# bkomuves/plonky2-verifier

Hardware: AMD Instinct MI355X
Metric: Plonky2 proofs verified/sec (std config, 28 FRI queries) at 1/2/4/8 MI355X (higher is better)
Workload: dtype u64 (Goldilocks mod-p integer)

## Files before the change

plonky2-verifier_amd/csrc/api_internal.hpp:

```cpp
#pragma once
#include <hip/hip_runtime.h>
#include <atomic>
#include <memory>
#include <mutex>
#include <string>
#include <utility>
#include <vector>
#include "../../include/p2v.h"
#include "circuit.hpp"
#include "dev.h"

using namespace p2v;

#pragma GCC visibility push(hidden)
extern thread_local std::string g_err;
inline int fail(int code, const std::string& msg) { g_err = msg; return code; }

template <class F>
int guarded(int other, F fn) {
  try { fn(); return P2V_OK; }
  catch (const ShapeError& e) { return fail(P2V_E_SHAPE, e.what()); }
  catch (const ParseError& e) { return fail(P2V_E_PARSE, e.what()); }
  catch (const CircuitError& e) { return fail(P2V_E_CIRCUIT, e.what()); }
  catch (const std::exception& e) { return fail(other, e.what()); }
// ... 65 lines not shown
  mutable std::vector<HostPipe*> pool;
  mutable std::mutex known_mu;
  mutable std::vector<std::unique_ptr<KnownTable>> known;
  ~p2v_circuit();
};

struct p2v_verifier {
  const p2v_circuit* circ = nullptr;
  int device = 0;
  size_t max_batch = 0, Bmax = 0;
  DevCircuit dc{};
  size_t in_bytes = 0;
  std::atomic<bool> p1_recorded{false};
  p2v_verifier* chain_prev = nullptr;
  std::vector<p2v_verifier*> chain_next;
  unsigned la_seq = 0;
  float last_ms[kNumKernels] = {0};
  bool timed = false;
  int transcript_mode = 0;
  int quad_min_batch = 4096;
  int lane_min_batch = 16384;
  bool merkle_cse = true;
  bool cse_dirty = false;
  int known_mode = 1;
  const KnownTable* known = nullptr;
  bool known_dirty = false;
  int lat_max_batch = 64;
  bool single_stream = false;
  bool debug_sync = false;
  ProofTemplate tmpl;
  bool have_tmpl = false;
  int64_t skel_len = 0, ntok = 0;
  bool have_bmap = false;
  int nruns = 0, nchk = 0;
  int64_t bfixed = 0;

  PinnedBuf h_res;
  Event ev[2 * kNumKernels];
  Event dep_p1, dep_side, dep_fri, dep_v3;
  Event p1_done;
  Event tr_done[2], chal_free[2];
  Stream side;
  Stream side2;
  Stream ts;
  Stream side3;
  DevBuf kid;
// ... 44 lines not shown
```

plonky2-verifier_amd/csrc/api_run.cpp:

```cpp
#include <algorithm>
#include <cstdio>
#include <cstring>
#include "api_internal.hpp"
#include "kernels.h"

extern "C" {

size_t p2v_tiled_words(size_t n, size_t proof_words) { return (n + 63) / 64 * 64 * proof_words; }

void p2v_tile_proofs(const uint64_t* pm, size_t n, size_t W, uint64_t* tiled) {
  if (!pm || !tiled) return;
  const size_t tiles = (n + 63) / 64;
  for (size_t t = 0; t < tiles; t++) {
    uint64_t* dst = tiled + t * W * 64;
    for (size_t w = 0; w < W; w++)
      for (size_t l = 0; l < 64; l++) {
        const size_t i = t * 64 + l;
        dst[w * 64 + l] = i < n ? pm[i * W + w] : 0;
      }
  }
}

static void launch_phase1(const DevCircuit& d, int tl, int nt_blocks, int leaf_blocks, hipStream_t s) {
  auto* k = d.key_id ? (tl == 1 ? k_phase1_lane_keyed : k_phase1_keyed) : (tl == 1 ? k_phase1_lane : k_phase1);
  k<<<nt_blocks + leaf_blocks, 256, 0, s>>>(d, nt_blocks, tl);
}
static void launch_transcript(const DevCircuit& d, int tl, int nt_blocks, hipStream_t s) {
  auto* k = d.key_id ? (tl == 1 ? k_transcript_lane_keyed : k_transcript_keyed) : (tl == 1 ? k_transcript_lane : k_transcript);
  k<<<nt_blocks, 256, 0, s>>>(d, tl);
}
static void launch_vanish(void (*k)(DevCircuit), int first, int last, int NPB, hipStream_t s, const DevCircuit& d) {
  k<<<(last - first) * NPB, 64, 0, s>>>(d);
}

int p2v_verifier_run(p2v_verifier* v, const uint64_t* proofs, size_t n, int8_t* results, uint64_t* trace, void* stream_, uint32_t flags) {
  return p2v_verifier_run_keyed(v, proofs, nullptr, n, results, trace, stream_, flags);
}

int p2v_verifier_run_keyed(p2v_verifier* v, const uint64_t* proofs, const uint32_t* key_ids, size_t n, int8_t* results,
                           uint64_t* trace, void* stream_, uint32_t flags) {
  if (!v || (!proofs && n) || !results) return fail(P2V_E_ARG, "null argument");
  if (n > v->max_batch) return fail(P2V_E_ARG, "batch larger than max_batch");
  if (n == 0) return P2V_OK;
  HCK(hipSetDevice(v->device));
  hipStream_t st = (hipStream_t)stream_;
  const Circuit& C = v->circ->c;
  DevCircuit d = v->dc;
  d.n = (int)n;
// ... 28 lines not shown
  d.soa = src;
  int tl = d.B >= v->lane_min_batch ? 1 : d.B >= v->quad_min_batch ? 4 : 16;
  if (v->transcript_mode == 1) tl = 16;
  else if (v->transcript_mode == 2) tl = 4;
  else if (v->transcript_mode == 3) tl = 1;
  const int nt_blocks = (tl * d.B + 255) / 256;
  const bool lat = d.n <= v->lat_max_batch;
  const bool key_rows = !key_ids || (d.nkeys > 1 && v->known && v->known->kkeys == d.nkeys);
  if (v->known && key_rows && !lat && d.mcse) {
    d.kmode = v->known_mode; d.kskip = 1;
    int k = 0;
    for (int j = 0; j < d.T; j++) if (v->dc.leaf_order[j] != 0) d.leaf_order[k++] = v->dc.leaf_order[j];
    d.nleaf = k;
  }
  const int leaf_units = d.Q * d.nleaf * NPB;
  bool chained = false;
  {
    std::lock_guard<std::mutex> lk(g_chain_mu);
    chained = v->chain_prev != nullptr;
    if (v->chain_prev && v->chain_prev->p1_recorded.load(std::memory_order_acquire))
      HCK(hipStreamWaitEvent(st, v->chain_prev->p1_done, 0));
  }
  const bool la = (flags & P2V_FLAG_LOOKAHEAD) && (flags & P2V_FLAG_INPUT_DEVICE) && sd != st && !chained;
  int la_slot = 0;
  if (la) {
    if (!v->ts) HCK(v->ts.create());
    la_slot = (int)(v->la_seq++ & 1u);
    d.chal = (uint64_t*)(la_slot ? v->chal2.p : v->chal.p);
    HCK(hipStreamWaitEvent(v->ts, v->chal_free[la_slot], 0));
    T0(SLOT_TRANSCRIPT, v->ts);
    launch_transcript(d, tl, nt_blocks, v->ts);
    DBG("k_transcript", v->ts);
    T1(SLOT_TRANSCRIPT, v->ts);
    HCK(hipEventRecord(v->tr_done[la_slot], v->ts));
    T0(SLOT_LEAF, st);
    k_leaf<<<(leaf_units + 3) / 4, 256, 0, st>>>(d);
    DBG("k_leaf", st);
    T1(SLOT_LEAF, st);
    HCK(hipStreamWaitEvent(st, v->tr_done[la_slot], 0));
    HCK(hipEventRecord(v->dep_p1, st));
    HCK(hipStreamWaitEvent(sd, v->dep_p1, 0));
  } else {
    T0(SLOT_PHASE1, st);
    launch_phase1(d, tl, nt_blocks, (leaf_units + 3) / 4, st);
    DBG("k_phase1", st);
    T1(SLOT_PHASE1, st);
    if (sd != st) {
      HCK(hipEventRecord(v->dep_p1, st));
      HCK(hipStreamWaitEvent(sd, v->dep_p1, 0));
    }
  }
  HCK(hipEventRecord(v->p1_done, st));
  v->p1_recorded.store(true, std::memory_order_release);
  const int mk_wg = lat ? 64 : 256;
  const bool fri2 = lat && sd != st;
  if (fri2 && !v->side2) HCK(v->side2.create());
  if (fri2) {
    HCK(hipStreamWaitEvent(v->side2, v->p1_done, 0));
    T0(SLOT_FRI, v->side2);
    k_fri<<<(d.Q * NPB * 64 + mk_wg - 1) / mk_wg, mk_wg, 0, v->side2>>>(d);
    DBG("k_fri", v->side2);
    T1(SLOT_FRI, v->side2);
    HCK(hipEventRecord(v->dep_fri, v->side2));
  }
  if (d.kmode) {
    if (v->known_dirty) HCK(hipMemsetAsync(v->k_missn.p, 0, 64, sd));
    v->known_dirty = true;
// ... 27 lines not shown
    HCK(hipEventRecord(v->dep_v3, sv));
    HCK(hipStreamWaitEvent(sd, v->dep_v3, 0));
  }
  if (d.vcls[4] > d.vcls[3]) launch_vanish(r2 ? k_vanish_lookup_r2 : k_vanish_lookup_rn, d.vcls[3], d.vcls[4], NPB, sd, d);
  DBG("k_vanish_lookup", sd);
  if (d.vcls[5] > d.vcls[4]) launch_vanish(r2 ? k_vanish_prog_r2 : k_vanish_prog_rn, d.vcls[4], d.vcls[5], NPB, sd, d);
  DBG("k_vanish_prog", sd);
  T1(SLOT_VANISH, sd);
  T0(SLOT_VANISH_FINAL, sd);
  k_vanish_final<<<(d.B + 255) / 256, 256, 0, sd>>>(d);
  DBG("k_vanish_final", sd);
  T1(SLOT_VANISH_FINAL, sd);
  if (!fri2) {
    T0(SLOT_FRI, sd);
    k_fri<<<(d.Q * NPB * 64 + 255) / 256, 256, 0, sd>>>(d);
    DBG("k_fri", sd);
    T1(SLOT_FRI, sd);
  }
  if (sd != st) HCK(hipEventRecord(v->dep_side, sd));
  T0(SLOT_MERKLE, st);
  const int merkle_units = d.Q * d.T * NPB;
  if (lat) k_merkle_row<<<(unsigned)(((int64_t)d.Q * d.T * d.n * 16 + 255) / 256), 256, 0, st>>>(d);
  else if (d.mcse) {
    const int ncls = 1 + d.S;
    if (v->cse_dirty) HCK(hipMemsetAsync(v->m_count.p, 0, (size_t)(d.depth0 + 2) * 64, st));
    v->cse_dirty = true;
    k_merkle_plan<<<(ncls * d.Q * NPB + P2V_PLAN_WAVES - 1) / P2V_PLAN_WAVES, 64 * P2V_PLAN_WAVES, 0, st>>>(d);
    DBG("k_merkle_plan", st);
    const int64_t cse_waves = ((int64_t)(d.T - d.kskip) * d.Q * d.n + 63) / 64 + d.depth0 + 1;
    k_merkle_cse<<<(unsigned)((cse_waves + 31) / 32 * 8), 256, 0, st>>>(d);
    DBG("k_merkle_cse", st);
    k_merkle_fix<<<P2V_FIX_BLOCKS, 256, 0, st>>>(d);
    DBG("k_merkle_fix", st);
    k_merkle_resolve<<<(d.Q * (d.T - d.kskip) * NPB + 3) / 4, 256, 0, st>>>(d);
    DBG("k_merkle_resolve", st);
    v->cse_dirty = false;
  } else k_merkle<<<(merkle_units + 3) / 4, 256, 0, st>>>(d);
  DBG("k_merkle", st);
  T1(SLOT_MERKLE, st);
  if (sd != st) HCK(hipStreamWaitEvent(st, v->dep_side, 0));
  if (fri2) HCK(hipStreamWaitEvent(st, v->dep_fri, 0));
  T0(SLOT_STATUS, st);
  k_status<<<(unsigned)((n + 255) / 256), 256, 0, st>>>(d, dres, dtrace, C.trace_words);
  DBG("k_status", st);
  T1(SLOT_STATUS, st);
  v->known_dirty = false;
  if (la) HCK(hipEventRecord(v->chal_free[la_slot], st));
  else if (sd != st) HCK(hipEventRecord(v->chal_free[0], st));
#undef T0
#undef T1
#undef DBG
// ... 29 lines not shown
```

plonky2-verifier_amd/csrc/api_workspace.cpp:

```cpp
#include <algorithm>
#include <cstdlib>
#include <cstring>
#include "api_internal.hpp"
#include "gl.h"
#include "poseidon_constants.h"

std::mutex g_chain_mu;


void fill_scalars(const Circuit& C, DevCircuit& d) {
  d.r = C.r; d.Q = C.num_queries; d.S = (int)C.arities.size(); d.T = 4 + d.S;
  d.num_pis = C.num_pis; d.cap_len = C.cap_len; d.degree_bits = C.degree_bits; d.lde_bits = C.lde_bits; d.pow_bits = C.pow_bits;
  d.num_wires = C.num_wires; d.num_routed = C.num_routed; d.num_constants = C.num_constants; d.ngc = C.num_gate_consts;
  d.ngroups = (int)C.grp_start.size(); d.nls = C.nls; d.nlp = C.nlp; d.npp = C.npp; d.qdf = C.qdf; d.nluts = (int)C.lut_in.size();
  d.depth0 = C.depth0; d.final_len = C.final_len;
  for (int t = 0; t < 4; t++) { d.width[t] = C.oracle_width[t]; d.lwidth[t] = C.leaf_width[t]; }
  d.noop_leaves = C.noop_leaves ? 1 : 0;
  d.n_gates = C.n_gate_eval; d.n_pp_terms = (int)C.n_pp_terms_per_round; d.n_lookup_terms = (int)C.n_lookup_terms_per_round;
  d.alpha_base_gates = C.alpha_base_gates;
  d.prog_pih = -1;
  const Layout& L = C.L;
  d.pis = L.pis; d.wcap = L.wcap; d.zcap = L.zcap; d.qcap = L.qcap; d.o_const = L.o_const; d.o_sig = L.o_sig; d.o_wires = L.o_wires;
  d.o_zs = L.o_zs; d.o_pp = L.o_pp; d.o_quot = L.o_quot; d.o_lzs = L.o_lzs; d.o_zs_next = L.o_zs_next; d.o_lzs_next = L.o_lzs_next;
  d.n_this = L.n_this; d.n_next = L.n_next; d.ccaps = L.ccaps; d.final_poly = L.final_poly; d.pow = L.pow; d.q0 = L.q0; d.qstride = L.qstride;
// ... 192 lines not shown
  }
  v->chain_prev = prev;
  if (prev) prev->chain_next.push_back(v);
  return P2V_OK;
}

int p2v_verifier_create(const p2v_circuit* pc, int device, size_t max_batch, p2v_verifier** out) {
  if (!pc || !out || max_batch == 0) return fail(P2V_E_ARG, "null argument / zero batch");
  if (const char* tm = getenv("P2V_TRANSCRIPT"); tm && !strcmp(tm, "pair"))
    return fail(P2V_E_ARG, "P2V_TRANSCRIPT=pair: the pair transcript form was retired (DESIGN.md §5.7)");
  int ndev = 0;
  if (hipGetDeviceCount(&ndev) != hipSuccess || ndev == 0) return fail(P2V_E_NODEVICE, "no HIP device available: libp2v verifies on MI355X only (no CPU fallback)");
  if (device < 0 || device >= ndev) return fail(P2V_E_ARG, "bad device index");
  HCK(hipSetDevice(device));
  const Circuit& C = pc->c;
  VerifierPtr v(new p2v_verifier());
  v->circ = pc; v->device = device; v->max_batch = max_batch;
  v->Bmax = (max_batch + 63) / 64 * 64;
  if (const char* ss = getenv("P2V_SINGLE_STREAM")) v->single_stream = ss[0] == '1';
  if (const char* ds = getenv("P2V_DEBUG_SYNC")) v->debug_sync = ds[0] == '1';
  if (const char* lm = getenv("P2V_LANE_MIN")) v->lane_min_batch = atoi(lm) > 0 ? atoi(lm) : v->lane_min_batch;
  if (const char* qm = getenv("P2V_QUAD_MIN")) v->quad_min_batch = atoi(qm) > 0 ? atoi(qm) : v->quad_min_batch;
  if (const char* mc = getenv("P2V_MERKLE_CSE")) v->merkle_cse = mc[0] != '0';
  if (const char* kl = getenv("P2V_KNOWN_LEAVES")) v->known_mode = kl[0] == '0' ? 0 : kl[0] == '2' ? 2 : 1;
  if (const char* lx = getenv("P2V_LAT_MAX")) v->lat_max_batch = atoi(lx) >= 0 ? atoi(lx) : v->lat_max_batch;
  if (const char* tm = getenv("P2V_TRANSCRIPT")) v->transcript_mode = !strcmp(tm, "row") ? 1 : !strcmp(tm, "quad") ? 2 : !strcmp(tm, "lane") ? 3 : 0;
  DevCircuit& d = v->dc;
  memset(&d, 0, sizeof d);
  fill_scalars(C, d);
  const CircuitTables t = circuit_tables(C);
  d.n_lut_pieces = t.pbase.back();
#define ACK(x) HCK_AS("device allocation", x)
  {
    std::vector<uint64_t> keys(C.cs_cap);
    keys.insert(keys.end(), C.digest, C.digest + 4);
    keys.insert(keys.end(), C.extra_keys.begin(), C.extra_keys.end());
    keys.insert(keys.end(), 8, 0);
    ACK(upload(v->t_cs, keys, d.keys));
    d.cs_cap = d.keys;
    d.nkeys = (int32_t)C.num_keys();
  }
  ACK(v->kid.alloc(v->Bmax * sizeof(uint32_t)));
  ACK(upload(v->t_kis, C.k_is, d.k_is));
  ACK(upload(v->t_gkind, t.gkind, d.gate_kind)); ACK(upload(v->t_gpar, t.gpar, d.gate_par)); ACK(upload(v->t_ggrp, t.ggrp, d.gate_grp));
  ACK(upload(v->t_gwoff, t.gwoff, d.gate_woff)); ACK(upload(v->t_w, t.wts, d.weights)); ACK(upload(v->t_gs, t.gs, d.grp_start)); ACK(upload(v->t_ge, t.ge, d.grp_end));
  ACK(upload(v->t_lin, t.lin, d.lut_in)); ACK(upload(v->t_lout, t.lout, d.lut_out)); ACK(upload(v->t_loff, t.loff, d.lut_off)); ACK(upload(v->t_llen, t.llen, d.lut_len));
// ... 85 lines not shown
```

plonky2-verifier_amd/csrc/dev.h:

```cpp
#pragma once
#include <stdint.h>

#define P2V_MAX_STEPS 8
#define P2V_MAX_R 4
#define P2V_LUT_CHUNK 16
#define P2V_LUT_PIECE 256
#define P2V_PLAN_WAVES 16
#define P2V_FIX_BLOCKS 256

struct DevCircuit {
  int32_t B;
  int32_t n;
  int32_t r, Q, S, T;
  int32_t num_pis, cap_len, degree_bits, lde_bits, pow_bits;
  int32_t num_wires, num_routed, num_constants, ngc, ngroups, nls, nlp, npp, qdf, nluts;
  int32_t depth0, final_len;
  int32_t arity[P2V_MAX_STEPS], step_depth[P2V_MAX_STEPS], step_logn[P2V_MAX_STEPS];
  int32_t width[4];
  int32_t lwidth[4];
  int32_t noop_leaves;
  int32_t tiled;
  int64_t wstride;
  int8_t leaf_order[4 + P2V_MAX_STEPS], merkle_order[4 + P2V_MAX_STEPS];
  int32_t n_gates;
  int32_t unit_filters;
  int32_t n_pp_terms, n_lookup_terms;
  int64_t alpha_base_gates;
  int64_t pis, wcap, zcap, qcap, o_const, o_sig, o_wires, o_zs, o_pp, o_quot, o_lzs, o_zs_next, o_lzs_next;
  int64_t n_this, n_next, ccaps, final_poly, pow, q0, qstride;
  int64_t leaf[4], path[4], step_evals[P2V_MAX_STEPS], step_path[P2V_MAX_STEPS];
// ... 123 lines not shown
```

plonky2-verifier_amd/csrc/kernels.h:

```cpp
#pragma once
#include <hip/hip_runtime.h>
#include <cstdint>
#include "dev.h"

extern "C" __global__ void k_phase1(DevCircuit, int, int);
extern "C" __global__ void k_phase1_lane(DevCircuit, int, int);
extern "C" __global__ void k_transcript(DevCircuit, int);
extern "C" __global__ void k_transcript_lane(DevCircuit, int);
extern "C" __global__ void k_phase1_keyed(DevCircuit, int, int);
extern "C" __global__ void k_phase1_lane_keyed(DevCircuit, int, int);
extern "C" __global__ void k_transcript_keyed(DevCircuit, int);
extern "C" __global__ void k_transcript_lane_keyed(DevCircuit, int);
extern "C" __global__ void k_leaf(DevCircuit);
extern "C" __global__ void k_fri(DevCircuit);
extern "C" __global__ void k_status(DevCircuit, int8_t*, uint64_t*, int64_t);
extern "C" __global__ void k_selftest(int, const uint64_t*, const uint64_t*, uint64_t*, int64_t);
extern "C" __global__ void k_selftest_forms(int, const uint64_t*, uint64_t*, int64_t);
extern "C" __global__ void k_selftest_field(int, DevCircuit, const uint64_t*, uint64_t*);
extern "C" __global__ void k_merkle(DevCircuit);
extern "C" __global__ void k_merkle_row(DevCircuit);
extern "C" __global__ void k_merkle_plan(DevCircuit);
extern "C" __global__ void k_merkle_cse(DevCircuit);
extern "C" __global__ void k_merkle_fix(DevCircuit);
extern "C" __global__ void k_merkle_resolve(DevCircuit);
extern "C" __global__ void k_merkle_known(DevCircuit);
extern "C" __global__ void k_merkle_known_miss(DevCircuit);
extern "C" __global__ void k_vanish_r2(DevCircuit);
extern "C" __global__ void k_vanish_rn(DevCircuit);
extern "C" __global__ void k_vanish_poseidon_r2(DevCircuit);
extern "C" __global__ void k_vanish_poseidon_rn(DevCircuit);
extern "C" __global__ void k_vanish_coset_r2(DevCircuit);
extern "C" __global__ void k_vanish_coset_rn(DevCircuit);
extern "C" __global__ void k_vanish_lookup_r2(DevCircuit);
// ... 12 lines not shown
```

plonky2-verifier_amd/csrc/kernels.hip:

```cpp
#include "leafhash.h"
#include "kernels.h"

using namespace p2d;
using gl::E;

__device__ __forceinline__ void leaf_hash_unit(const DevCircuit& c, int unit, int lane) {
  const int NPB = c.B >> 6;
  const int pb = unit % NPB, qt = unit / NPB;
  const int q = qt % c.Q, t = c.leaf_order[qt / c.Q];
  const int p = pb * 64 + lane;
  const int64_t base = c.q0 + (int64_t)q * c.qstride;
  int64_t off; int len;
  if (t < 4) { off = base + c.leaf[t]; len = c.lwidth[t]; }
  else { int s = t - 4; off = base + c.step_evals[s]; len = 2 << c.arity[s]; }
  uint64_t st[12];
  leaf_sponge(c, off, len, p, st);
  uint64_t* dst = c.leafdig + ((int64_t)(q * c.T + t) * 4) * c.B + p;
#pragma unroll
  for (int i = 0; i < 4; i++) dst[(int64_t)i * c.B] = st[i];
}

template <int D>
__device__ __forceinline__ uint64_t row_up(uint64_t v, bool plus) {
  const uint32_t lo = (uint32_t)v, hi = (uint32_t)(v >> 32);
// ... 166 lines not shown
      uint64_t w = f.get_word(x, outpos);
      outpos--;
      if (type == TOP_SQUEEZE_IDX) w &= qmask;
      if (a + k == CH_FRI_ALPHA(c)) fa0 = w;
      if (a + k == CH_FRI_ALPHA(c) + 1) fa1 = w;
      if (leader) chal(c, a + k, p) = w;
    }
  }
  E ap[F::LOG + 1] = {E{fa0, fa1}};
#pragma unroll
  for (int s = 1; s <= F::LOG; s++) ap[s] = gl::emul(ap[s - 1], ap[s - 1]);
  E H[2];
#pragma unroll
  for (int b = 0; b < 2 * F::SUMS_FIRST; b++) H[b] = horner_strided<1 << F::LOG>(c, b == 0 ? c.o_const : c.o_zs_next, b == 0 ? c.n_this : c.n_next, f.t, p, ap[F::LOG]);
#pragma unroll
  for (int b = 0; b < 2; b++) {
    if constexpr (!F::SUMS_FIRST) H[b] = horner_strided<1 << F::LOG>(c, b == 0 ? c.o_const : c.o_zs_next, b == 0 ? c.n_this : c.n_next, f.t, p, ap[F::LOG]);
    const E y = f.fold(H[b], ap);
    if (leader) { chal(c, (b == 0 ? CH_Y0(c) : CH_Y1(c)), p) = y.a; chal(c, (b == 0 ? CH_Y0(c) : CH_Y1(c)) + 1, p) = y.b; }
  }
}

template <int FORM = 0, bool KEYED = false>
__device__ __forceinline__ void transcript_block(const DevCircuit& c, int tl, TLdsAny& U) {
  const int g = blockIdx.x * 256 + threadIdx.x;
  if constexpr (FORM == 1) {
    if (g < c.B) transcript<KEYED>(c, g, LaneForm{});
  } else if (tl == 16) {
    lp::Row LR;
    lp::init(LR, U.l, threadIdx.x);
    if ((g >> 4) < c.B) transcript<KEYED>(c, g >> 4, RowForm(LR, U.l));
  } else {
    if ((g >> 2) < c.B) transcript<KEYED>(c, g >> 2, QuadForm{g & 3, U.q});
  }
}

template <int FORM, bool KEYED = false>
__device__ __forceinline__ void phase1_body(const DevCircuit& c, int nt_blocks, int tl) {
  const int lane = threadIdx.x & 63, wave = threadIdx.x >> 6;
  __shared__ TLdsAny T;
  if ((int)blockIdx.x < nt_blocks) {
    __builtin_amdgcn_s_setprio(3);
    if constexpr (FORM == 0) tlds_fill_form(T, tl);
    transcript_block<FORM, KEYED>(c, tl, T);
    return;
  }
  const int unit = ((int)blockIdx.x - nt_blocks) * 4 + wave;
  const int units = c.Q * c.nleaf * (c.B >> 6);
  if (unit < units) leaf_hash_unit(c, unit, lane);
}
extern "C" __global__ void __launch_bounds__(256) __attribute__((amdgpu_waves_per_eu(4))) k_phase1(DevCircuit c, int nt_blocks, int tl) {
  phase1_body<0>(c, nt_blocks, tl);
}
extern "C" __global__ void __launch_bounds__(256) __attribute__((amdgpu_waves_per_eu(4))) k_phase1_lane(DevCircuit c, int nt_blocks, int tl) {
  phase1_body<1>(c, nt_blocks, tl);
}
extern "C" __global__ void __launch_bounds__(256) __attribute__((amdgpu_waves_per_eu(4))) k_phase1_keyed(DevCircuit c, int nt_blocks, int tl) {
  phase1_body<0, true>(c, nt_blocks, tl);
}
extern "C" __global__ void __launch_bounds__(256) __attribute__((amdgpu_waves_per_eu(4))) k_phase1_lane_keyed(DevCircuit c, int nt_blocks, int tl) {
  phase1_body<1, true>(c, nt_blocks, tl);
}

extern "C" __global__ void __launch_bounds__(256) k_transcript(DevCircuit c, int tl) {
  __builtin_amdgcn_s_setprio(3);
  __shared__ TLdsAny T;
  tlds_fill_form(T, tl);
  transcript_block(c, tl, T);
}
extern "C" __global__ void __launch_bounds__(256) k_transcript_lane(DevCircuit c, int tl) {
  __builtin_amdgcn_s_setprio(3);
  __shared__ TLdsAny T;
  transcript_block<1>(c, tl, T);
}
extern "C" __global__ void __launch_bounds__(256) k_transcript_keyed(DevCircuit c, int tl) {
  __builtin_amdgcn_s_setprio(3);
  __shared__ TLdsAny T;
  tlds_fill_form(T, tl);
  transcript_block<0, true>(c, tl, T);
}
extern "C" __global__ void __launch_bounds__(256) k_transcript_lane_keyed(DevCircuit c, int tl) {
  __builtin_amdgcn_s_setprio(3);
  __shared__ TLdsAny T;
  transcript_block<1, true>(c, tl, T);
// ... 358 lines not shown
```

plonky2-verifier_amd/csrc/merkle.hip:

```cpp
#include "leafhash.h"
#include "kernels.h"

using namespace p2d;

__device__ __forceinline__ uint32_t entry_pack(int t, int q, int p) { return (uint32_t)t << 27 | (uint32_t)q << 22 | (uint32_t)p; }
__device__ __forceinline__ void entry_unpack(uint32_t id, int& t, int& q, int& p) {
  t = (int)(id >> 27); q = (int)((id >> 22) & 31); p = (int)(id & 0x3FFFFFu);
}
__device__ __forceinline__ uint32_t plan_pack(int e, int owner, bool same_leaf, int root) {
  return (uint32_t)e | (uint32_t)owner << 4 | (uint32_t)same_leaf << 9 | (uint32_t)root << 10;
}
__device__ __forceinline__ int plan_e(uint32_t pw) { return (int)(pw & 15); }
__device__ __forceinline__ int plan_owner(uint32_t pw) { return (int)((pw >> 4) & 31); }
__device__ __forceinline__ bool plan_same_leaf(uint32_t pw) { return (pw >> 9) & 1; }
__device__ __forceinline__ int plan_root(uint32_t pw) { return (int)((pw >> 10) & 31); }
__device__ __forceinline__ uint8_t& mk_at(const DevCircuit& c, int t, int q, int p) { return c.mk_ok[(int64_t)(q * c.T + t) * c.B + p]; }

#ifndef P2V_MERKLE_WAVES
#define P2V_MERKLE_WAVES 6
#endif
#if P2V_MERKLE_WAVES > 0
#define P2V_MERKLE_ATTR __attribute__((amdgpu_waves_per_eu(P2V_MERKLE_WAVES)))
#else
#define P2V_MERKLE_ATTR
#endif
__device__ __forceinline__ void tree_path(const DevCircuit& c, int t, int q, int p, int& depth, int64_t& poff, uint32_t& idx) {
  const int64_t base = c.q0 + (int64_t)q * c.qstride;
  idx = (uint32_t)chal(c, CH_QIDX(c) + q, p);
  if (t < 4) { depth = c.depth0; poff = base + c.path[t]; }
  else {
    const int s = t - 4;
    int sh = 0;
    for (int j = 0; j <= s; j++) sh += c.arity[j];
    idx >>= sh; depth = c.step_depth[s]; poff = base + c.step_path[s];
  }
}
__device__ __forceinline__ void load_leafdig(const DevCircuit& c, int t, int q, int p, uint64_t (&cur)[4]) {
  const uint64_t* src = c.leafdig + ((int64_t)(q * c.T + t) * 4) * c.B + p;
#pragma unroll
// ... 58 lines not shown
  return ok && (rp::get_word(eq, 0) & rp::get_word(eq, 1) & rp::get_word(eq, 2) & rp::get_word(eq, 3));
}

__device__ __forceinline__ bool path_ok(const DevCircuit& c, int t, int q, int p) {
  int depth; int64_t poff; uint32_t idx;
  tree_path(c, t, q, p, depth, poff, idx);
  uint64_t cur[4];
  load_leafdig(c, t, q, p, cur);
  lane_climb(c, poff, 0, depth, p, cur, idx);
  return cap_ok(c, t, idx, cur, p);
}
__device__ __forceinline__ void merkle_unit(const DevCircuit& c) {
  const int lane = threadIdx.x & 63;
  const int unit = blockIdx.x * 4 + (threadIdx.x >> 6);
  const int NPB = c.B >> 6;
  if (unit >= c.Q * c.T * NPB) return;
  const int pb = unit % NPB, qt = unit / NPB;
  const int q = qt % c.Q, t = c.merkle_order[qt / c.Q];
  const int p = pb * 64 + lane;
  mk_at(c, t, q, p) = path_ok(c, t, q, p) ? 1 : 0;
}
extern "C" __global__ void __launch_bounds__(256) P2V_MERKLE_ATTR k_merkle(DevCircuit c) { merkle_unit(c); }

#define P2V_CSE_CSTRIDE 16
__device__ __forceinline__ void class_shape(const DevCircuit& c, int cls, int& sh, int& depth) {
  sh = 0; depth = c.depth0;
  if (cls > 0) { for (int j = 0; j < cls; j++) sh += c.arity[j]; depth = c.step_depth[cls - 1]; }
}
__device__ __forceinline__ int tree_class(int t) { return t < 4 ? 0 : t - 3; }
__device__ __forceinline__ int64_t plan_at(const DevCircuit& c, int t, int q, int p) { return ((int64_t)tree_class(t) * c.Q + q) * c.B + p; }
extern "C" __global__ void __launch_bounds__(64 * P2V_PLAN_WAVES) k_merkle_plan(DevCircuit c) {
  __shared__ int hist[P2V_CSE_MAX_DEPTH + 1], gbase[P2V_CSE_MAX_DEPTH + 1];
  const int lane = threadIdx.x & 63;
  const int unit = blockIdx.x * P2V_PLAN_WAVES + (threadIdx.x >> 6);
  const int NPB = c.B >> 6, ncls = 1 + c.S;
  const int nb = c.depth0 + 1;
  if (threadIdx.x < (unsigned)nb) hist[threadIdx.x] = 0;
  __syncthreads();
  const bool unit_live = unit < ncls * c.Q * NPB;
  const int pb = unit % NPB, cq = unit / NPB;
  const int q = cq % c.Q, cls = unit_live ? cq / c.Q : 0;
  const int p = pb * 64 + lane;
  const bool live = unit_live && p < c.n;
  int sh, depth;
  class_shape(c, cls, sh, depth);
  const int ntr = cls == 0 ? 4 - c.kskip : 1, t0 = cls == 0 ? c.kskip : 3 + cls;
  int e = 0, loc = 0, cnt = 0;
  if (live) {
    const uint64_t* qi = c.chal + (int64_t)CH_QIDX(c) * c.B + p;
    const uint32_t me = (uint32_t)qi[(int64_t)q * c.B] >> sh;
    int minb = 64, owner = q, root = q;
    bool have_root = false;
    uint64_t fol = ~0ULL;
    for (int k0 = 0; k0 < c.Q; k0 += 4) {
      uint32_t ik[4];
#pragma unroll
      for (int u = 0; u < 4; u++) ik[u] = k0 + u < c.Q ? (uint32_t)qi[(int64_t)(k0 + u) * c.B] >> sh : me;
#pragma unroll
      for (int u = 0; u < 4; u++) {
        const int k = k0 + u;
        if (k >= c.Q) break;
        const uint32_t x = me ^ ik[u];
        const int b = x ? 32 - __clz(x) : 0;
        if (!have_root && b <= depth) { root = k; have_root = true; }
        if (k < q) {
          if (b < minb) { minb = b; owner = k; }
        } else if (k > q && b >= 1 && b <= depth) {
          const int sl = 5 * (b - 1);
          if (((fol >> sl) & 31) == 31) fol ^= (uint64_t)(31 ^ k) << sl;
        }
      }
    }
    e = minb - 1 >= depth ? depth : (minb >= 1 ? minb - 1 : 0);
    if (e < depth) fol |= ~0ULL << (5 * e);
    const int64_t pi = ((int64_t)cls * c.Q + q) * c.B + p;
    c.mplan[pi] = plan_pack(e, owner, minb == 0, root);
    c.mfol[pi] = fol;
    for (int tt = 0; tt < ntr; tt++) {
      c.mbadq[((int64_t)(t0 + tt) * c.Q + q) * c.B + p] = 0;
      mk_at(c, t0 + tt, q, p) = 0;
    }
  }
  uint64_t todo = __ballot(live);
  while (todo) {
    const int lead = __ffsll((unsigned long long)todo) - 1;
    const int eb = __shfl(e, lead);
    const uint64_t grp = __ballot(live && e == eb);
    const int n = __popcll(grp);
    int off = 0;
    if (lane == lead) off = atomicAdd(&hist[eb], n * ntr);
    off = __shfl(off, lead);
    if (live && e == eb) { loc = off + __popcll(grp & ((1ULL << lane) - 1)); cnt = n; }
    todo &= ~grp;
  }
  __syncthreads();
  if (threadIdx.x < (unsigned)nb) {
    const int h = hist[threadIdx.x];
    gbase[threadIdx.x] = h ? atomicAdd(&c.mcount[threadIdx.x * P2V_CSE_CSTRIDE], h) : 0;
  }
  __syncthreads();
  if (live) {
    uint32_t* dst = c.mchain + (int64_t)e * c.mcap;
    const int64_t base = (int64_t)gbase[e] + loc;
    for (int tt = 0; tt < ntr; tt++) {
      const int64_t pos = base + (int64_t)tt * cnt;
      if (pos < c.mcap) dst[pos] = entry_pack(t0 + tt, q, p);
    }
  }
}
__device__ __forceinline__ bool cse_flag_once(const DevCircuit& c, int t, int q, int p) {
  const size_t at = ((size_t)t * c.Q + q) * c.B + p;
  uint32_t* w = (uint32_t*)(c.mbadq + (at & ~(size_t)3));
  const uint32_t bit = 1u << (8 * (at & 3));
  return !(atomicOr(w, bit) & bit);
}
__device__ __forceinline__ void cse_flag(const DevCircuit& c, int t, int q, int p) {
  if (!cse_flag_once(c, t, q, p)) return;
  const int at = atomicAdd(c.mfixn, 1);
  if (at < c.mcap) c.mfix[at] = entry_pack(t, q, p);
  else mk_at(c, t, q, p) = 0;
}
__device__ __forceinline__ bool cse_wave(const DevCircuit& c, int& b, int64_t& w) {
  const int nbk = c.depth0 + 1;
  uint64_t nw[P2V_CSE_MAX_DEPTH + 1];
  uint64_t total = 0;
#pragma unroll
  for (int k = 0; k <= P2V_CSE_MAX_DEPTH; k++) {
    nw[k] = k < nbk ? ((uint64_t)min((int64_t)c.mcount[k * P2V_CSE_CSTRIDE], c.mcap) + 63) >> 6 : 0;
    total += nw[k];
  }
  const int wv = __builtin_amdgcn_readfirstlane((int)(threadIdx.x >> 6));
// ... 296 lines not shown
```

Before: 1.603 million.

## Restructure Merkle plan into LDS-tiled per-proof routine, optionally fused into phase1

Moves the Merkle CSE planning logic into a shared header that stages query indices for a tile of proofs in LDS and computes plans per proof. The routine runs in two passes: one builds a histogram, the second recomputes the level and places chain entries. The standalone plan kernel now uses this routine over groups of proofs. An env-gated option (off by default) also runs it at the end of each phase1 transcript block, which drops one launch but adds LDS pressure and syncs to phase1. The m_count reset is moved earlier so it runs before phase1.

```diff
diff --git a/plonky2-verifier_amd/csrc/api_internal.hpp b/plonky2-verifier_amd/csrc/api_internal.hpp
--- a/plonky2-verifier_amd/csrc/api_internal.hpp
+++ b/plonky2-verifier_amd/csrc/api_internal.hpp
@@ -111,6 +111,7 @@
   int lane_min_batch = 16384;
   bool merkle_cse = true;
   bool cse_dirty = false;
+  bool plan_fused = false;
   int known_mode = 1;
   const KnownTable* known = nullptr;
   bool known_dirty = false;
diff --git a/plonky2-verifier_amd/csrc/api_run.cpp b/plonky2-verifier_amd/csrc/api_run.cpp
--- a/plonky2-verifier_amd/csrc/api_run.cpp
+++ b/plonky2-verifier_amd/csrc/api_run.cpp
@@ -21,9 +21,9 @@
   }
 }
 
-static void launch_phase1(const DevCircuit& d, int tl, int nt_blocks, int leaf_blocks, hipStream_t s) {
+static void launch_phase1(const DevCircuit& d, int tl, int nt_blocks, int leaf_blocks, bool plan, hipStream_t s) {
   auto* k = d.key_id ? (tl == 1 ? k_phase1_lane_keyed : k_phase1_keyed) : (tl == 1 ? k_phase1_lane : k_phase1);
-  k<<<nt_blocks + leaf_blocks, 256, 0, s>>>(d, nt_blocks, tl);
+  k<<<nt_blocks + leaf_blocks, 256, 0, s>>>(d, nt_blocks, tl, plan ? 1 : 0);
 }
 static void launch_transcript(const DevCircuit& d, int tl, int nt_blocks, hipStream_t s) {
   auto* k = d.key_id ? (tl == 1 ? k_transcript_lane_keyed : k_transcript_keyed) : (tl == 1 ? k_transcript_lane : k_transcript);
@@ -98,6 +98,12 @@
       HCK(hipStreamWaitEvent(st, v->chain_prev->p1_done, 0));
   }
   const bool la = (flags & P2V_FLAG_LOOKAHEAD) && (flags & P2V_FLAG_INPUT_DEVICE) && sd != st && !chained;
+  const bool cse = !lat && d.mcse;
+  const bool plan_p1 = cse && !la && v->plan_fused;
+  if (cse) {
+    if (v->cse_dirty) HCK(hipMemsetAsync(v->m_count.p, 0, (size_t)(d.depth0 + 2) * 64, st));
+    v->cse_dirty = true;
+  }
   int la_slot = 0;
   if (la) {
     if (!v->ts) HCK(v->ts.create());
@@ -118,7 +124,7 @@
     HCK(hipStreamWaitEvent(sd, v->dep_p1, 0));
   } else {
     T0(SLOT_PHASE1, st);
-    launch_phase1(d, tl, nt_blocks, (leaf_units + 3) / 4, st);
+    launch_phase1(d, tl, nt_blocks, (leaf_units + 3) / 4, plan_p1, st);
     DBG("k_phase1", st);
     T1(SLOT_PHASE1, st);
     if (sd != st) {
@@ -192,11 +198,10 @@
   const int merkle_units = d.Q * d.T * NPB;
   if (lat) k_merkle_row<<<(unsigned)(((int64_t)d.Q * d.T * d.n * 16 + 255) / 256), 256, 0, st>>>(d);
   else if (d.mcse) {
-    const int ncls = 1 + d.S;
-    if (v->cse_dirty) HCK(hipMemsetAsync(v->m_count.p, 0, (size_t)(d.depth0 + 2) * 64, st));
-    v->cse_dirty = true;
-    k_merkle_plan<<<(ncls * d.Q * NPB + P2V_PLAN_WAVES - 1) / P2V_PLAN_WAVES, 64 * P2V_PLAN_WAVES, 0, st>>>(d);
-    DBG("k_merkle_plan", st);
+    if (!plan_p1) {
+      k_merkle_plan<<<(d.n + P2V_PLAN_PROOFS - 1) / P2V_PLAN_PROOFS, 64 * P2V_PLAN_WAVES, 0, st>>>(d);
+      DBG("k_merkle_plan", st);
+    }
     const int64_t cse_waves = ((int64_t)(d.T - d.kskip) * d.Q * d.n + 63) / 64 + d.depth0 + 1;
     k_merkle_cse<<<(unsigned)((cse_waves + 31) / 32 * 8), 256, 0, st>>>(d);
     DBG("k_merkle_cse", st);
diff --git a/plonky2-verifier_amd/csrc/api_workspace.cpp b/plonky2-verifier_amd/csrc/api_workspace.cpp
--- a/plonky2-verifier_amd/csrc/api_workspace.cpp
+++ b/plonky2-verifier_amd/csrc/api_workspace.cpp
@@ -238,6 +238,7 @@
   if (const char* lm = getenv("P2V_LANE_MIN")) v->lane_min_batch = atoi(lm) > 0 ? atoi(lm) : v->lane_min_batch;
   if (const char* qm = getenv("P2V_QUAD_MIN")) v->quad_min_batch = atoi(qm) > 0 ? atoi(qm) : v->quad_min_batch;
   if (const char* mc = getenv("P2V_MERKLE_CSE")) v->merkle_cse = mc[0] != '0';
+  if (const char* pf = getenv("P2V_PLAN_FUSED")) v->plan_fused = pf[0] != '0';
   if (const char* kl = getenv("P2V_KNOWN_LEAVES")) v->known_mode = kl[0] == '0' ? 0 : kl[0] == '2' ? 2 : 1;
   if (const char* lx = getenv("P2V_LAT_MAX")) v->lat_max_batch = atoi(lx) >= 0 ? atoi(lx) : v->lat_max_batch;
   if (const char* tm = getenv("P2V_TRANSCRIPT")) v->transcript_mode = !strcmp(tm, "row") ? 1 : !strcmp(tm, "quad") ? 2 : !strcmp(tm, "lane") ? 3 : 0;
diff --git a/plonky2-verifier_amd/csrc/dev.h b/plonky2-verifier_amd/csrc/dev.h
--- a/plonky2-verifier_amd/csrc/dev.h
+++ b/plonky2-verifier_amd/csrc/dev.h
@@ -6,6 +6,7 @@
 #define P2V_LUT_CHUNK 16
 #define P2V_LUT_PIECE 256
 #define P2V_PLAN_WAVES 16
+#define P2V_PLAN_PROOFS 16
 #define P2V_FIX_BLOCKS 256
 
 struct DevCircuit {
diff --git a/plonky2-verifier_amd/csrc/kernels.h b/plonky2-verifier_amd/csrc/kernels.h
--- a/plonky2-verifier_amd/csrc/kernels.h
+++ b/plonky2-verifier_amd/csrc/kernels.h
@@ -3,12 +3,12 @@
 #include <cstdint>
 #include "dev.h"
 
-extern "C" __global__ void k_phase1(DevCircuit, int, int);
-extern "C" __global__ void k_phase1_lane(DevCircuit, int, int);
+extern "C" __global__ void k_phase1(DevCircuit, int, int, int);
+extern "C" __global__ void k_phase1_lane(DevCircuit, int, int, int);
 extern "C" __global__ void k_transcript(DevCircuit, int);
 extern "C" __global__ void k_transcript_lane(DevCircuit, int);
-extern "C" __global__ void k_phase1_keyed(DevCircuit, int, int);
-extern "C" __global__ void k_phase1_lane_keyed(DevCircuit, int, int);
+extern "C" __global__ void k_phase1_keyed(DevCircuit, int, int, int);
+extern "C" __global__ void k_phase1_lane_keyed(DevCircuit, int, int, int);
 extern "C" __global__ void k_transcript_keyed(DevCircuit, int);
 extern "C" __global__ void k_transcript_lane_keyed(DevCircuit, int);
 extern "C" __global__ void k_leaf(DevCircuit);
diff --git a/plonky2-verifier_amd/csrc/kernels.hip b/plonky2-verifier_amd/csrc/kernels.hip
--- a/plonky2-verifier_amd/csrc/kernels.hip
+++ b/plonky2-verifier_amd/csrc/kernels.hip
@@ -1,4 +1,5 @@
 #include "leafhash.h"
+#include "merkle_plan.h"
 #include "kernels.h"
 
 using namespace p2d;
@@ -212,44 +213,61 @@
 }
 
 template <int FORM = 0, bool KEYED = false>
-__device__ __forceinline__ void transcript_block(const DevCircuit& c, int tl, TLdsAny& U) {
+__device__ __forceinline__ int transcript_block(const DevCircuit& c, int tl, TLdsAny& U) {
   const int g = blockIdx.x * 256 + threadIdx.x;
   if constexpr (FORM == 1) {
-    if (g < c.B) transcript<KEYED>(c, g, LaneForm{});
+    int p = g;
+    asm volatile("" : "+v"(p));
+    if (p < c.B) transcript<KEYED>(c, p, LaneForm{});
+    return p & 255;
   } else if (tl == 16) {
     lp::Row LR;
     lp::init(LR, U.l, threadIdx.x);
-    if ((g >> 4) < c.B) transcript<KEYED>(c, g >> 4, RowForm(LR, U.l));
+    int p = g >> 4;
+    asm volatile("" : "+v"(p));
+    if (p < c.B) transcript<KEYED>(c, p, RowForm(LR, U.l));
+    return (p << 4 | LR.L) & 255;
   } else {
-    if ((g >> 2) < c.B) transcript<KEYED>(c, g >> 2, QuadForm{g & 3, U.q});
+    int p = g >> 2;
+    asm volatile("" : "+v"(p));
+    const int t = g & 3;
+    if (p < c.B) transcript<KEYED>(c, p, QuadForm{t, U.q});
+    return (p << 2 | t) & 255;
   }
 }
 
 template <int FORM, bool KEYED = false>
-__device__ __forceinline__ void phase1_body(const DevCircuit& c, int nt_blocks, int tl) {
+__device__ __forceinline__ void phase1_body(const DevCircuit& c, int nt_blocks, int tl, int plan) {
   const int lane = threadIdx.x & 63, wave = threadIdx.x >> 6;
-  __shared__ TLdsAny T;
+  __shared__ union { TLdsAny t; PlanLds pl; } U;
+  TLdsAny& T = U.t;
   if ((int)blockIdx.x < nt_blocks) {
     __builtin_amdgcn_s_setprio(3);
     if constexpr (FORM == 0) tlds_fill_form(T, tl);
-    transcript_block<FORM, KEYED>(c, tl, T);
+    const int tid = transcript_block<FORM, KEYED>(c, tl, T);
+    if (plan) {
+      __threadfence_block();
+      __syncthreads();
+      const int np = 256 / (FORM == 1 ? 1 : tl);
+      merkle_plan_proofs(c, (int)blockIdx.x * np, np, tid, U.pl);
+    }
     return;
   }
   const int unit = ((int)blockIdx.x - nt_blocks) * 4 + wave;
   const int units = c.Q * c.nleaf * (c.B >> 6);
   if (unit < units) leaf_hash_unit(c, unit, lane);
 }
-extern "C" __global__ void __launch_bounds__(256) __attribute__((amdgpu_waves_per_eu(4))) k_phase1(DevCircuit c, int nt_blocks, int tl) {
-  phase1_body<0>(c, nt_blocks, tl);
-}
-extern "C" __global__ void __launch_bounds__(256) __attribute__((amdgpu_waves_per_eu(4))) k_phase1_lane(DevCircuit c, int nt_blocks, int tl) {
-  phase1_body<1>(c, nt_blocks, tl);
-}
-extern "C" __global__ void __launch_bounds__(256) __attribute__((amdgpu_waves_per_eu(4))) k_phase1_keyed(DevCircuit c, int nt_blocks, int tl) {
-  phase1_body<0, true>(c, nt_blocks, tl);
-}
-extern "C" __global__ void __launch_bounds__(256) __attribute__((amdgpu_waves_per_eu(4))) k_phase1_lane_keyed(DevCircuit c, int nt_blocks, int tl) {
-  phase1_body<1, true>(c, nt_blocks, tl);
+extern "C" __global__ void __launch_bounds__(256) __attribute__((amdgpu_waves_per_eu(4))) k_phase1(DevCircuit c, int nt_blocks, int tl, int plan) {
+  phase1_body<0>(c, nt_blocks, tl, plan);
+}
+extern "C" __global__ void __launch_bounds__(256) __attribute__((amdgpu_waves_per_eu(4))) k_phase1_lane(DevCircuit c, int nt_blocks, int tl, int plan) {
+  phase1_body<1>(c, nt_blocks, tl, plan);
+}
+extern "C" __global__ void __launch_bounds__(256) __attribute__((amdgpu_waves_per_eu(4))) k_phase1_keyed(DevCircuit c, int nt_blocks, int tl, int plan) {
+  phase1_body<0, true>(c, nt_blocks, tl, plan);
+}
+extern "C" __global__ void __launch_bounds__(256) __attribute__((amdgpu_waves_per_eu(4))) k_phase1_lane_keyed(DevCircuit c, int nt_blocks, int tl, int plan) {
+  phase1_body<1, true>(c, nt_blocks, tl, plan);
 }
 
 extern "C" __global__ void __launch_bounds__(256) k_transcript(DevCircuit c, int tl) {
diff --git a/plonky2-verifier_amd/csrc/merkle.hip b/plonky2-verifier_amd/csrc/merkle.hip
--- a/plonky2-verifier_amd/csrc/merkle.hip
+++ b/plonky2-verifier_amd/csrc/merkle.hip
@@ -1,20 +1,8 @@
 #include "leafhash.h"
+#include "merkle_plan.h"
 #include "kernels.h"
 
 using namespace p2d;
-
-__device__ __forceinline__ uint32_t entry_pack(int t, int q, int p) { return (uint32_t)t << 27 | (uint32_t)q << 22 | (uint32_t)p; }
-__device__ __forceinline__ void entry_unpack(uint32_t id, int& t, int& q, int& p) {
-  t = (int)(id >> 27); q = (int)((id >> 22) & 31); p = (int)(id & 0x3FFFFFu);
-}
-__device__ __forceinline__ uint32_t plan_pack(int e, int owner, bool same_leaf, int root) {
-  return (uint32_t)e | (uint32_t)owner << 4 | (uint32_t)same_leaf << 9 | (uint32_t)root << 10;
-}
-__device__ __forceinline__ int plan_e(uint32_t pw) { return (int)(pw & 15); }
-__device__ __forceinline__ int plan_owner(uint32_t pw) { return (int)((pw >> 4) & 31); }
-__device__ __forceinline__ bool plan_same_leaf(uint32_t pw) { return (pw >> 9) & 1; }
-__device__ __forceinline__ int plan_root(uint32_t pw) { return (int)((pw >> 10) & 31); }
-__device__ __forceinline__ uint8_t& mk_at(const DevCircuit& c, int t, int q, int p) { return c.mk_ok[(int64_t)(q * c.T + t) * c.B + p]; }
 
 #ifndef P2V_MERKLE_WAVES
 #define P2V_MERKLE_WAVES 6
@@ -119,91 +107,9 @@
 }
 extern "C" __global__ void __launch_bounds__(256) P2V_MERKLE_ATTR k_merkle(DevCircuit c) { merkle_unit(c); }
 
-#define P2V_CSE_CSTRIDE 16
-__device__ __forceinline__ void class_shape(const DevCircuit& c, int cls, int& sh, int& depth) {
-  sh = 0; depth = c.depth0;
-  if (cls > 0) { for (int j = 0; j < cls; j++) sh += c.arity[j]; depth = c.step_depth[cls - 1]; }
-}
-__device__ __forceinline__ int tree_class(int t) { return t < 4 ? 0 : t - 3; }
-__device__ __forceinline__ int64_t plan_at(const DevCircuit& c, int t, int q, int p) { return ((int64_t)tree_class(t) * c.Q + q) * c.B + p; }
 extern "C" __global__ void __launch_bounds__(64 * P2V_PLAN_WAVES) k_merkle_plan(DevCircuit c) {
-  __shared__ int hist[P2V_CSE_MAX_DEPTH + 1], gbase[P2V_CSE_MAX_DEPTH + 1];
-  const int lane = threadIdx.x & 63;
-  const int unit = blockIdx.x * P2V_PLAN_WAVES + (threadIdx.x >> 6);
-  const int NPB = c.B >> 6, ncls = 1 + c.S;
-  const int nb = c.depth0 + 1;
-  if (threadIdx.x < (unsigned)nb) hist[threadIdx.x] = 0;
-  __syncthreads();
-  const bool unit_live = unit < ncls * c.Q * NPB;
-  const int pb = unit % NPB, cq = unit / NPB;
-  const int q = cq % c.Q, cls = unit_live ? cq / c.Q : 0;
-  const int p = pb * 64 + lane;
-  const bool live = unit_live && p < c.n;
-  int sh, depth;
-  class_shape(c, cls, sh, depth);
-  const int ntr = cls == 0 ? 4 - c.kskip : 1, t0 = cls == 0 ? c.kskip : 3 + cls;
-  int e = 0, loc = 0, cnt = 0;
-  if (live) {
-    const uint64_t* qi = c.chal + (int64_t)CH_QIDX(c) * c.B + p;
-    const uint32_t me = (uint32_t)qi[(int64_t)q * c.B] >> sh;
-    int minb = 64, owner = q, root = q;
-    bool have_root = false;
-    uint64_t fol = ~0ULL;
-    for (int k0 = 0; k0 < c.Q; k0 += 4) {
-      uint32_t ik[4];
-#pragma unroll
-      for (int u = 0; u < 4; u++) ik[u] = k0 + u < c.Q ? (uint32_t)qi[(int64_t)(k0 + u) * c.B] >> sh : me;
-#pragma unroll
-      for (int u = 0; u < 4; u++) {
-        const int k = k0 + u;
-        if (k >= c.Q) break;
-        const uint32_t x = me ^ ik[u];
-        const int b = x ? 32 - __clz(x) : 0;
-        if (!have_root && b <= depth) { root = k; have_root = true; }
-        if (k < q) {
-          if (b < minb) { minb = b; owner = k; }
-        } else if (k > q && b >= 1 && b <= depth) {
-          const int sl = 5 * (b - 1);
-          if (((fol >> sl) & 31) == 31) fol ^= (uint64_t)(31 ^ k) << sl;
-        }
-      }
-    }
-    e = minb - 1 >= depth ? depth : (minb >= 1 ? minb - 1 : 0);
-    if (e < depth) fol |= ~0ULL << (5 * e);
-    const int64_t pi = ((int64_t)cls * c.Q + q) * c.B + p;
-    c.mplan[pi] = plan_pack(e, owner, minb == 0, root);
-    c.mfol[pi] = fol;
-    for (int tt = 0; tt < ntr; tt++) {
-      c.mbadq[((int64_t)(t0 + tt) * c.Q + q) * c.B + p] = 0;
-      mk_at(c, t0 + tt, q, p) = 0;
-    }
-  }
-  uint64_t todo = __ballot(live);
-  while (todo) {
-    const int lead = __ffsll((unsigned long long)todo) - 1;
-    const int eb = __shfl(e, lead);
-    const uint64_t grp = __ballot(live && e == eb);
-    const int n = __popcll(grp);
-    int off = 0;
-    if (lane == lead) off = atomicAdd(&hist[eb], n * ntr);
-    off = __shfl(off, lead);
-    if (live && e == eb) { loc = off + __popcll(grp & ((1ULL << lane) - 1)); cnt = n; }
-    todo &= ~grp;
-  }
-  __syncthreads();
-  if (threadIdx.x < (unsigned)nb) {
-    const int h = hist[threadIdx.x];
-    gbase[threadIdx.x] = h ? atomicAdd(&c.mcount[threadIdx.x * P2V_CSE_CSTRIDE], h) : 0;
-  }
-  __syncthreads();
-  if (live) {
-    uint32_t* dst = c.mchain + (int64_t)e * c.mcap;
-    const int64_t base = (int64_t)gbase[e] + loc;
-    for (int tt = 0; tt < ntr; tt++) {
-      const int64_t pos = base + (int64_t)tt * cnt;
-      if (pos < c.mcap) dst[pos] = entry_pack(t0 + tt, q, p);
-    }
-  }
+  __shared__ PlanLds L;
+  merkle_plan_proofs(c, (int)blockIdx.x * P2V_PLAN_PROOFS, P2V_PLAN_PROOFS, (int)threadIdx.x, L);
 }
 __device__ __forceinline__ bool cse_flag_once(const DevCircuit& c, int t, int q, int p) {
   const size_t at = ((size_t)t * c.Q + q) * c.B + p;
diff --git a/plonky2-verifier_amd/csrc/merkle_plan.h b/plonky2-verifier_amd/csrc/merkle_plan.h
--- /dev/null
+++ b/plonky2-verifier_amd/csrc/merkle_plan.h
@@ -0,0 +1,145 @@
+#pragma once
+#include "devcommon.h"
+
+namespace p2d {
+
+__device__ __forceinline__ uint32_t entry_pack(int t, int q, int p) { return (uint32_t)t << 27 | (uint32_t)q << 22 | (uint32_t)p; }
+__device__ __forceinline__ void entry_unpack(uint32_t id, int& t, int& q, int& p) {
+  t = (int)(id >> 27); q = (int)((id >> 22) & 31); p = (int)(id & 0x3FFFFFu);
+}
+__device__ __forceinline__ uint32_t plan_pack(int e, int owner, bool same_leaf, int root) {
+  return (uint32_t)e | (uint32_t)owner << 4 | (uint32_t)same_leaf << 9 | (uint32_t)root << 10;
+}
+__device__ __forceinline__ int plan_e(uint32_t pw) { return (int)(pw & 15); }
+__device__ __forceinline__ int plan_owner(uint32_t pw) { return (int)((pw >> 4) & 31); }
+__device__ __forceinline__ bool plan_same_leaf(uint32_t pw) { return (pw >> 9) & 1; }
+__device__ __forceinline__ int plan_root(uint32_t pw) { return (int)((pw >> 10) & 31); }
+__device__ __forceinline__ uint8_t& mk_at(const DevCircuit& c, int t, int q, int p) { return c.mk_ok[(int64_t)(q * c.T + t) * c.B + p]; }
+
+#define P2V_CSE_CSTRIDE 16
+__device__ __forceinline__ void class_shape(const DevCircuit& c, int cls, int& sh, int& depth) {
+  sh = 0; depth = c.depth0;
+  if (cls > 0) { for (int j = 0; j < cls; j++) sh += c.arity[j]; depth = c.step_depth[cls - 1]; }
+}
+__device__ __forceinline__ int tree_class(int t) { return t < 4 ? 0 : t - 3; }
+__device__ __forceinline__ int64_t plan_at(const DevCircuit& c, int t, int q, int p) { return ((int64_t)tree_class(t) * c.Q + q) * c.B + p; }
+__device__ __forceinline__ void class_trees(const DevCircuit& c, int cls, int& t0, int& ntr) {
+  ntr = cls == 0 ? 4 - c.kskip : 1; t0 = cls == 0 ? c.kskip : 3 + cls;
+}
+
+#define P2V_PLAN_TILE 64
+struct PlanLds {
+  uint32_t idx[P2V_CSE_MAX_Q][P2V_PLAN_TILE];
+  int hist[P2V_CSE_MAX_DEPTH + 1], gbase[P2V_CSE_MAX_DEPTH + 1];
+};
+
+__device__ __forceinline__ int plan_levels(int minb, int depth) { return minb - 1 >= depth ? depth : (minb >= 1 ? minb - 1 : 0); }
+__device__ __forceinline__ int plan_e_of(const DevCircuit& c, const PlanLds& L, int q, int j, int sh, int depth) {
+  const uint32_t me = L.idx[q][j] >> sh;
+  int minb = 64;
+  for (int k = 0; k < q; k++) {
+    const uint32_t x = me ^ (L.idx[k][j] >> sh);
+    minb = min(minb, x ? 32 - __clz(x) : 0);
+  }
+  return plan_levels(minb, depth);
+}
+__device__ __forceinline__ int plan_unit(const DevCircuit& c, const PlanLds& L, int cls, int q, int p, int j) {
+  int sh, depth, t0, ntr;
+  class_shape(c, cls, sh, depth);
+  class_trees(c, cls, t0, ntr);
+  const uint32_t me = L.idx[q][j] >> sh;
+  int minb = 64, owner = q, root = q;
+  bool have_root = false;
+  uint64_t fol = ~0ULL;
+  for (int k = 0; k < c.Q; k++) {
+    const uint32_t x = me ^ (L.idx[k][j] >> sh);
+    const int b = x ? 32 - __clz(x) : 0;
+    if (!have_root && b <= depth) { root = k; have_root = true; }
+    if (k < q) {
+      if (b < minb) { minb = b; owner = k; }
+    } else if (k > q && b >= 1 && b <= depth) {
+      const int sl = 5 * (b - 1);
+      if (((fol >> sl) & 31) == 31) fol ^= (uint64_t)(31 ^ k) << sl;
+    }
+  }
+  const int e = plan_levels(minb, depth);
+  if (e < depth) fol |= ~0ULL << (5 * e);
+  const int64_t pi = ((int64_t)cls * c.Q + q) * c.B + p;
+  c.mplan[pi] = plan_pack(e, owner, minb == 0, root);
+  c.mfol[pi] = fol;
+  for (int tt = 0; tt < ntr; tt++) {
+    c.mbadq[((int64_t)(t0 + tt) * c.Q + q) * c.B + p] = 0;
+    mk_at(c, t0 + tt, q, p) = 0;
+  }
+  return e;
+}
+template <bool PLACE>
+__device__ __forceinline__ void plan_runs(PlanLds& L, int lane, bool live, int e, int ntr, int& loc, int& cnt) {
+  const int key = e << 3 | ntr;
+  uint64_t todo = __ballot(live);
+  while (todo) {
+    const int lead = __ffsll((unsigned long long)todo) - 1;
+    const int kb = __shfl(key, lead);
+    const uint64_t grp = __ballot(live && key == kb);
+    const int n = __popcll(grp);
+    int off = 0;
+    if (lane == lead) off = atomicAdd(&L.hist[kb >> 3], n * (kb & 7));
+    if constexpr (PLACE) {
+      off = __shfl(off, lead);
+      if (live && key == kb) { loc = off + __popcll(grp & ((1ULL << lane) - 1)); cnt = n; }
+    }
+    todo &= ~grp;
+  }
+}
+__device__ __forceinline__ void merkle_plan_proofs(const DevCircuit& c, int p0, int np, int tid, PlanLds& L) {
+  const int nb = c.depth0 + 1, nth = (int)blockDim.x;
+  for (int pt = p0; pt < p0 + np && pt < c.n; pt += P2V_PLAN_TILE) {
+    const int tn = min(P2V_PLAN_TILE, p0 + np - pt);
+    const int items = tn * (1 + c.S) * c.Q;
+    __syncthreads();
+    for (int i = tid; i < tn * c.Q; i += nth) {
+      const int q = i / tn, j = i - q * tn;
+      L.idx[q][j] = pt + j < c.n ? (uint32_t)chal(c, CH_QIDX(c) + q, pt + j) : 0;
+    }
+    if (tid < nb) L.hist[tid] = 0;
+    __syncthreads();
+    for (int i0 = 0; i0 < items; i0 += nth) {
+      const int item = i0 + tid;
+      const int u = item / tn, j = item - u * tn, p = pt + j;
+      const bool live = item < items && p < c.n;
+      const int cls = live ? u / c.Q : 0, q = live ? u % c.Q : 0;
+      int t0, ntr, loc, cnt;
+      class_trees(c, cls, t0, ntr);
+      const int e = live ? plan_unit(c, L, cls, q, p, j) : 0;
+      plan_runs<false>(L, tid & 63, live, e, ntr, loc, cnt);
+    }
+    __syncthreads();
+    if (tid < nb) {
+      const int h = L.hist[tid];
+      L.gbase[tid] = h ? atomicAdd(&c.mcount[tid * P2V_CSE_CSTRIDE], h) : 0;
+      L.hist[tid] = 0;
+    }
+    __syncthreads();
+    for (int i0 = 0; i0 < items; i0 += nth) {
+      const int item = i0 + tid;
+      const int u = item / tn, j = item - u * tn, p = pt + j;
+      const bool live = item < items && p < c.n;
+      const int cls = live ? u / c.Q : 0, q = live ? u % c.Q : 0;
+      int sh, depth, t0, ntr, loc = 0, cnt = 0;
+      class_shape(c, cls, sh, depth);
+      class_trees(c, cls, t0, ntr);
+      const int e = live ? plan_e_of(c, L, q, j, sh, depth) : 0;
+      plan_runs<true>(L, tid & 63, live, e, ntr, loc, cnt);
+      if (live) {
+        uint32_t* dst = c.mchain + (int64_t)e * c.mcap;
+        const int64_t base = (int64_t)L.gbase[e] + loc;
+        for (int tt = 0; tt < ntr; tt++) {
+          const int64_t pos = base + (int64_t)tt * cnt;
+          if (pos < c.mcap) dst[pos] = entry_pack(t0 + tt, q, p);
+        }
+      }
+    }
+  }
+}
+
+}
```

After: 1.609 million (median of 6 runs). Within noise of the previous version (+0.4%).
